# philipturner/metal-flash-attention

Hardware: NVIDIA H100
Metric: giga-FMA-instr/sec forward attn N=4096 D=128 bf16 (higher is better)
Workload: dtype bf16

## Files before the change

### metal-flash-attention_b200/csrc/kernels/sm90_ptx.cuh

```cuda
#pragma once
#include <cuda_runtime.h>
#include <stdint.h>

namespace mfa {
namespace ptx {

__device__ __forceinline__ uint32_t smem_u32(const void *p) { return static_cast<uint32_t>(__cvta_generic_to_shared(p)); }

__device__ __forceinline__ void mbar_init(uint64_t *bar, uint32_t count) {
  asm volatile("mbarrier.init.shared::cta.b64 [%0], %1;" ::"r"(smem_u32(bar)), "r"(count) : "memory");
}
__device__ __forceinline__ void fence_barrier_init() { asm volatile("fence.mbarrier_init.release.cluster;" ::: "memory"); }
__device__ __forceinline__ void fence_proxy_async_smem() { asm volatile("fence.proxy.async.shared::cta;" ::: "memory"); }

__device__ __forceinline__ void mbar_arrive(uint64_t *bar) {
  asm volatile("mbarrier.arrive.shared::cta.b64 _, [%0];" ::"r"(smem_u32(bar)) : "memory");
}
__device__ __forceinline__ void mbar_arrive_expect_tx(uint64_t *bar, uint32_t bytes) {
  asm volatile("mbarrier.arrive.expect_tx.shared::cta.b64 _, [%0], %1;" ::"r"(smem_u32(bar)), "r"(bytes) : "memory");
}
__device__ __forceinline__ void mbar_complete_tx(uint64_t *bar, uint32_t bytes) {
  asm volatile("mbarrier.complete_tx.relaxed.cta.shared::cta.b64 [%0], %1;" ::"r"(smem_u32(bar)), "r"(bytes) : "memory");
}
__device__ __forceinline__ bool mbar_try_wait(uint64_t *bar, uint32_t parity) {
  uint32_t ok;
  asm volatile(
      "{\n"
      ".reg .pred P;\n"
      "mbarrier.try_wait.parity.shared::cta.b64 P, [%1], %2;\n"
      "selp.u32 %0, 1, 0, P;\n"
      "}\n"
      : "=r"(ok)
      : "r"(smem_u32(bar)), "r"(parity)
      : "memory");
  return ok != 0;
}

#ifndef MFA_MBAR_TIMEOUT_CYCLES
#define MFA_MBAR_TIMEOUT_CYCLES (8000000000ll)
#endif
__device__ __forceinline__ void mbar_wait(uint64_t *bar, uint32_t parity) {
  if (mbar_try_wait(bar, parity)) return;
  const long long start = clock64();
  uint32_t spins = 0;
  while (!mbar_try_wait(bar, parity))
    if ((++spins & 0x3ffu) == 0 && clock64() - start > MFA_MBAR_TIMEOUT_CYCLES) __trap();
}

__device__ __forceinline__ void prefetch_tensormap(const void *map) {
  asm volatile("prefetch.tensormap [%0];" ::"l"(reinterpret_cast<uint64_t>(map)) : "memory");
}
__device__ __forceinline__ void tma_load_3d(void *smem_dst, const void *map, uint64_t *bar, int32_t c0, int32_t c1,
                                            int32_t c2) {
  asm volatile(
      "cp.async.bulk.tensor.3d.shared::cluster.global.mbarrier::complete_tx::bytes [%0], [%1, {%3, %4, %5}], [%2];"
      ::"r"(smem_u32(smem_dst)), "l"(reinterpret_cast<uint64_t>(map)), "r"(smem_u32(bar)), "r"(c0), "r"(c1), "r"(c2)
      : "memory");
}

__device__ __forceinline__ uint64_t make_smem_desc_sw128(uint32_t smem_addr, uint32_t lbo_bytes, uint32_t sbo_bytes) {
  uint64_t desc = 0;
  desc |= static_cast<uint64_t>((smem_addr & 0x3FFFFu) >> 4);
  desc |= static_cast<uint64_t>((lbo_bytes >> 4) & 0x3FFFu) << 16;
  desc |= static_cast<uint64_t>((sbo_bytes >> 4) & 0x3FFFu) << 32;
  desc |= static_cast<uint64_t>(1) << 62;
  return desc;
}

__device__ __forceinline__ float ex2_approx(float x) {
  float y;
  asm("ex2.approx.ftz.f32 %0, %1;" : "=f"(y) : "f"(x));
  return y;
}
__device__ __forceinline__ uint32_t pack_bf16x2(float lo, float hi) {
  uint32_t r;
  asm("cvt.rn.bf16x2.f32 %0, %1, %2;" : "=r"(r) : "f"(hi), "f"(lo));
  return r;
}
__device__ __forceinline__ uint32_t pack_f16x2(float lo, float hi) {
  uint32_t r;
  asm("cvt.rn.f16x2.f32 %0, %1, %2;" : "=r"(r) : "f"(hi), "f"(lo));
  return r;
}
__device__ __forceinline__ uint2 e4m3x4_to_f16x4(uint32_t bytes) {
  uint2 r;
  asm("{\n"
      ".reg .b16 lo, hi;\n"
      "mov.b32 {lo, hi}, %2;\n"
      "cvt.rn.f16x2.e4m3x2 %0, lo;\n"
      "cvt.rn.f16x2.e4m3x2 %1, hi;\n"
      "}\n"
      : "=r"(r.x), "=r"(r.y)
      : "r"(bytes));
  return r;
}
__device__ __forceinline__ uint32_t f16x2_to_bf16x2(uint32_t h) {
  float lo, hi;
  asm("{\n"
      ".reg .b16 a, b;\n"
      "mov.b32 {a, b}, %2;\n"
      "cvt.f32.f16 %0, a;\n"
      "cvt.f32.f16 %1, b;\n"
      "}\n"
      : "=f"(lo), "=f"(hi)
      : "r"(h));
  return pack_bf16x2(lo, hi);
}

}
}
```

### metal-flash-attention_b200/csrc/kernels/wgmma_attention.cu

```cuda
#include <cuda_fp16.h>
#include <cuda_runtime.h>
#include <math.h>
#include <stdint.h>

#include <type_traits>

#include "attention_params.h"
#include "backward_common.cuh"
#include "device_state.h"
#include "mfa_b200.h"
#include "sm90_ptx.cuh"
#include "tma_host.h"
#include "wgmma.cuh"

namespace mfa {
namespace hop {

using namespace ptx;
using bwd::load_16bit;
using bwd::load_stat;
using bwd::store_stat;

constexpr uint32_t kWG = 128;
constexpr uint32_t kRows = 64;
constexpr uint32_t kBarBytes = 64;

__device__ __forceinline__ uint32_t frag_row(uint32_t t) { return (t / 32) * 16 + (t % 32) / 4; }

template <uint32_t ROWS>
__device__ __forceinline__ uint64_t desc_kmajor(uint32_t tile, uint32_t row0, uint32_t kk) {
  return make_smem_desc_sw128(tile + (kk >> 2) * ROWS * 128 + row0 * 128 + (kk & 3) * 32, 16, 1024);
}
template <uint32_t ROWS>
__device__ __forceinline__ uint64_t desc_mnmajor(uint32_t tile, uint32_t kk, uint32_t c0) {
  return make_smem_desc_sw128(tile + c0 * ROWS * 128 + kk * 16 * 128, ROWS * 128, 1024);
}

template <uint32_t DCH, uint32_t N, bool kBF16, uint32_t ROWS_A>
__device__ __forceinline__ void mma_ss(float (&acc)[N / 2], uint32_t sA, uint32_t a0, uint32_t sB) {
#pragma unroll
  for (uint32_t kk = 0; kk < DCH * 4; ++kk)
    Wgmma<N, kBF16>::ss(acc, desc_kmajor<ROWS_A>(sA, a0, kk), desc_kmajor<N>(sB, 0, kk), kk > 0);
}

template <bool kBF16>
__device__ __forceinline__ uint32_t pack2(float lo, float hi) {
  return kBF16 ? pack_bf16x2(lo, hi) : pack_f16x2(lo, hi);
}
template <bool kBF16, int NR>
__device__ __forceinline__ void a_frag(const float (&s)[NR], uint32_t kk, uint32_t (&a)[4]) {
  a[0] = pack2<kBF16>(s[8 * kk + 0], s[8 * kk + 1]);
  a[1] = pack2<kBF16>(s[8 * kk + 2], s[8 * kk + 3]);
  a[2] = pack2<kBF16>(s[8 * kk + 4], s[8 * kk + 5]);
  a[3] = pack2<kBF16>(s[8 * kk + 6], s[8 * kk + 7]);
}

__device__ __forceinline__ uint8_t *align1024(uint8_t *p) {
  return reinterpret_cast<uint8_t *>((reinterpret_cast<uintptr_t>(p) + 1023) & ~uintptr_t(1023));
}

template <uint32_t RESIDENT, uint32_t TILE>
struct SmemLayout {
  static constexpr uint32_t kResidentBytes = RESIDENT, kStageBytes = 2 * TILE;
  static constexpr uint32_t kBarOffset = RESIDENT + 2 * kStageBytes;
  static constexpr uint32_t kSmemBytes = 1024 + kBarOffset + kBarBytes;
};

template <class Smem, bool kRelease = false>
struct Ring {
  uint8_t *base;
  uint64_t *bar;

  __device__ __forceinline__ explicit Ring(uint8_t *smem)
      : base(align1024(smem)), bar(reinterpret_cast<uint64_t *>(base + Smem::kBarOffset)) {}
  __device__ __forceinline__ uint8_t *stage(uint32_t n) const {
    return base + Smem::kResidentBytes + (n & 1) * Smem::kStageBytes;
  }

  __device__ __forceinline__ void init() const {
    if (threadIdx.x == 0) {
      for (int i = 0; i < 3; ++i) mbar_init(&bar[i], 1);
      if constexpr (kRelease)
        for (int i = 3; i < 5; ++i) mbar_init(&bar[i], 2);
      fence_barrier_init();
    }
    __syncthreads();
  }
  template <class Load>
  __device__ __forceinline__ void load(uint32_t n, uint32_t s, const Load &issue) const {
    mbar_arrive_expect_tx(&bar[1 + s], Smem::kStageBytes);
    issue(n, stage(s), &bar[1 + s]);
  }
  template <class Resident, class Load>
  __device__ __forceinline__ void start(const Resident &load_resident, uint32_t total, const Load &load) const {
    if (threadIdx.x != 0) return;
    mbar_arrive_expect_tx(&bar[0], Smem::kResidentBytes);
    load_resident(base, &bar[0]);
    for (uint32_t n = 0; n < 2 && n < total; ++n) this->load(n, n, load);
  }
  __device__ __forceinline__ void wait_resident() const { mbar_wait(&bar[0], 0); }
  __device__ __forceinline__ void wait(uint32_t n) const { mbar_wait(&bar[1 + (n & 1)], (n >> 1) & 1); }
  template <class Load>
  __device__ __forceinline__ void release_and_refill(uint32_t n, uint32_t total, const Load &load) const {
    __syncthreads();
    if (threadIdx.x == 0 && n + 2 < total) this->load(n + 2, n & 1, load);
  }
  __device__ __forceinline__ void release(uint32_t n) const {
    if (threadIdx.x % kWG == 0) mbar_arrive(&bar[3 + (n & 1)]);
  }
  template <class Load>
  __device__ __forceinline__ void refill(uint32_t n, uint32_t total, const Load &load) const {
    if (threadIdx.x == 0 && n + 2 < total) {
      mbar_wait(&bar[3 + (n & 1)], (n >> 1) & 1);
      this->load(n + 2, n & 1, load);
    }
  }
};

template <uint32_t DCH, uint32_t ROWS>
__device__ __forceinline__ void load_tile(uint8_t *dst, const CUtensorMap *map, uint64_t *bar, uint32_t row0,
                                          uint32_t head) {
#pragma unroll
  for (uint32_t c = 0; c < DCH; ++c) tma_load_3d(dst + c * ROWS * 128, map, bar, c * 64, row0, head);
}

template <int N>
__device__ __forceinline__ void zero(float (&d)[N]) {
#pragma unroll
  for (int i = 0; i < N; ++i) d[i] = 0.f;
}

template <uint32_t DCH, uint32_t ROWS, uint32_t kThreads>
__device__ __forceinline__ void zero_rows(uint8_t *tile, uint32_t first) {
  const uint32_t units = (ROWS - first) * 8;
  for (uint32_t i = threadIdx.x; i < DCH * units; i += kThreads) {
    const uint32_t c = i / units;
    reinterpret_cast<uint4 *>(tile + c * ROWS * 128 + first * 128)[i - c * units] = make_uint4(0u, 0u, 0u, 0u);
  }
}
template <uint32_t DCH, uint32_t ROWS, uint32_t kThreads>
__device__ __forceinline__ void zero_row_range(uint8_t *tile, uint32_t first, uint32_t end) {
  const uint32_t units = (end - first) * 8;
  for (uint32_t i = threadIdx.x; i < DCH * units; i += kThreads) {
    const uint32_t c = i / units;
    reinterpret_cast<uint4 *>(tile + c * ROWS * 128 + first * 128)[i - c * units] = make_uint4(0u, 0u, 0u, 0u);
  }
}

template <int NR>
__device__ __forceinline__ void store_acc(const float (&acc)[NR], float *out, uint32_t row0, uint32_t limit, uint32_t col0,
                                          uint32_t D, float inv0, float inv1) {
  const uint32_t t = threadIdx.x % kWG;
  const uint32_t r = row0 + frag_row(t);
#pragma unroll
  for (int i = 0; i < NR / 4; ++i) {
    const uint32_t col = col0 + 8 * i + 2 * (t % 4);
    if (col >= D) continue;
    if (r < limit)
      *reinterpret_cast<float2 *>(out + static_cast<size_t>(r) * D + col) = make_float2(acc[4 * i] * inv0, acc[4 * i + 1] * inv0);
    if (r + 8 < limit)
      *reinterpret_cast<float2 *>(out + static_cast<size_t>(r + 8) * D + col) =
          make_float2(acc[4 * i + 2] * inv1, acc[4 * i + 3] * inv1);
  }
}

template <uint32_t BN, bool kCausal>
__device__ __forceinline__ uint32_t key_blocks(uint32_t row_base, uint32_t rows, uint32_t R, uint32_t C, int delta,
                                               uint32_t kb0, uint32_t per_split) {
  if constexpr (!kCausal) {
    return min((C + BN - 1) / BN - kb0, per_split);
  } else {
    const int last_key = static_cast<int>(min(row_base + rows, R)) - 1 + delta;
    const int end = last_key < 0 ? 0 : min(static_cast<int>((C + BN - 1) / BN), last_key / static_cast<int>(BN) + 1);
    return static_cast<uint32_t>(max(0, min(end, static_cast<int>(kb0 + per_split)) - static_cast<int>(kb0)));
  }
}

template <uint32_t BM>
// ... 378 lines not shown
        first = kept.x * box;
        end = min(kept.y * box, end);
      }
      convert_fp8_kv<DCH, BN, Cfg::kThreads, kBF16>(ring.stage(j), ring.base + Cfg::Fp8Smem::kConvertedOffset, first, end);
      fence_proxy_async_smem();
      __syncthreads();
      if (tid == 0 && j + 2 < blocks) ring.load(j + 2, j & 1, load_kv);
    } else if constexpr (kLayout == KVLayout::kPaged && kBand) {
      const uint2 kept = band_boxes(kb0 + j, BN, box, band_lo, min(band_hi, static_cast<int>(span.C) - 1));
      const uint32_t first = kept.x * box, end = min(kept.y * box, span.C - (kb0 + j) * BN);
      if (first > 0 || end < BN) {
        zero_row_range<DCH, BN, Cfg::kThreads>(ring.stage(j), 0, first);
        zero_row_range<DCH, BN, Cfg::kThreads>(ring.stage(j), end, BN);
        zero_row_range<DCH, BN, Cfg::kThreads>(ring.stage(j) + Cfg::kKVBytes, 0, first);
        zero_row_range<DCH, BN, Cfg::kThreads>(ring.stage(j) + Cfg::kKVBytes, end, BN);
        fence_proxy_async_smem();
        __syncthreads();
      }
    } else if (kVarlen && ((kBand || kSplit ? kb0 : 0) + j + 1) * BN > span.C) {
      const uint32_t kb = (kBand || kSplit ? kb0 : 0) + j;
      zero_rows<DCH, BN, Cfg::kThreads>(ring.stage(j), span.C - kb * BN);
      zero_rows<DCH, BN, Cfg::kThreads>(ring.stage(j) + Cfg::kKVBytes, span.C - kb * BN);
      fence_proxy_async_smem();
      __syncthreads();
    }
    const uint32_t sK = smem_u32(kFp8 ? ring.base + Cfg::Fp8Smem::kConvertedOffset : ring.stage(j)), sV = sK + Cfg::kKVBytes;
    float sc[BN / 2];
    zero(sc);
    wgmma_fence();
    mma_ss<DCH, BN, kBF16, Cfg::kTileM>(sc, sQ, wg * kRows, sK);
    wgmma_commit();
    if constexpr (kRelease)
      if (j > 0) ring.refill(j - 1, blocks, load_kv);
    wgmma_wait<0>();
    fence_regs(sc);

    if ((kb0 + j + 1) * BN > span.C) mask_past_edge(sc, (kb0 + j) * BN, span.C);
    if constexpr (kSplit) {
      const int key0 = static_cast<int>((kb0 + j) * BN);
      const int64_t lower = kBand ? static_cast<int64_t>(delta) - band.left : -(int64_t(1) << 40);
      const int64_t upper = static_cast<int64_t>(delta) + (kBand ? band.right : 0);
      if ((kBand || kCausal) && crosses_band(key0, key0 + static_cast<int>(BN) - 1, static_cast<int>(row_base),
                                             static_cast<int>(row_base + tile_rows) - 1, lower, upper))
        mask_rows_outside_band(sc, qrow0, qrow1, key0, lower, upper);
    } else if constexpr (kBand) {
      const int key0 = static_cast<int>((kb0 + j) * BN), row = static_cast<int>(row_base + wg * kRows + frag_row(t));
      const int64_t lower = static_cast<int64_t>(delta) - band.left, upper = static_cast<int64_t>(delta) + band.right;
      if (crosses_band(key0, key0 + static_cast<int>(BN) - 1, static_cast<int>(row_base),
                       static_cast<int>(row_base + Cfg::kTileM) - 1, lower, upper))
        mask_outside_band<false>(sc, row, key0, lower, upper);
    } else if constexpr (kCausal) {
      const int key0 = static_cast<int>((kb0 + j) * BN);
      if (crosses_diagonal(key0 + static_cast<int>(BN) - 1, static_cast<int>(row_base), delta))
        mask_past_diagonal<false>(sc, static_cast<int>(row_base + wg * kRows + frag_row(t)), key0, delta);
    }
    float r0 = -INFINITY, r1 = -INFINITY;
#pragma unroll
    for (uint32_t i = 0; i < BN / 8; ++i) {
      r0 = fmaxf(r0, fmaxf(sc[4 * i], sc[4 * i + 1]));
      r1 = fmaxf(r1, fmaxf(sc[4 * i + 2], sc[4 * i + 3]));
    }
    r0 = fmaxf(r0, __shfl_xor_sync(0xffffffffu, r0, 1));
    r0 = fmaxf(r0, __shfl_xor_sync(0xffffffffu, r0, 2));
    r1 = fmaxf(r1, __shfl_xor_sync(0xffffffffu, r1, 1));
    r1 = fmaxf(r1, __shfl_xor_sync(0xffffffffu, r1, 2));
    const float mn0 = fmaxf(m0, r0 * scale_log2), mn1 = fmaxf(m1, r1 * scale_log2);
    const float ref0 = kCausal && mn0 == -INFINITY ? 0.f : mn0, ref1 = kCausal && mn1 == -INFINITY ? 0.f : mn1;
    const float a0 = ex2_approx(m0 - ref0), a1 = ex2_approx(m1 - ref1);
    m0 = mn0;
    m1 = mn1;
    l0 *= a0;
    l1 *= a1;
#pragma unroll
    for (uint32_t i = 0; i < NO / 8; ++i) {
      o[4 * i] *= a0;
      o[4 * i + 1] *= a0;
      o[4 * i + 2] *= a1;
      o[4 * i + 3] *= a1;
    }
#pragma unroll
    for (uint32_t i = 0; i < BN / 8; ++i) {
      sc[4 * i] = ex2_approx(fmaf(sc[4 * i], scale_log2, -ref0));
      sc[4 * i + 1] = ex2_approx(fmaf(sc[4 * i + 1], scale_log2, -ref0));
      sc[4 * i + 2] = ex2_approx(fmaf(sc[4 * i + 2], scale_log2, -ref1));
      sc[4 * i + 3] = ex2_approx(fmaf(sc[4 * i + 3], scale_log2, -ref1));
      l0 += sc[4 * i] + sc[4 * i + 1];
      l1 += sc[4 * i + 2] + sc[4 * i + 3];
    }
    wgmma_fence();
#pragma unroll
    for (uint32_t kk = 0; kk < BN / 16; ++kk) {
      uint32_t a[4];
      a_frag<kBF16>(sc, kk, a);
      Wgmma<NO, kBF16>::rs(o, a, desc_mnmajor<BN>(sV, kk, 0), 1);
      if constexpr (DCH == 1) {
        wgmma_commit();
        wgmma_wait<0>();
      }
    }
    wgmma_commit();
    wgmma_wait<0>();
    fence_regs(o);
    if constexpr (kFp8)
      __syncthreads();
    else if constexpr (kRelease)
      ring.release(j);
    else
      ring.release_and_refill(j, blocks, load_kv);
  }

  l0 += __shfl_xor_sync(0xffffffffu, l0, 1);
  l0 += __shfl_xor_sync(0xffffffffu, l0, 2);
  l1 += __shfl_xor_sync(0xffffffffu, l1, 1);
  l1 += __shfl_xor_sync(0xffffffffu, l1, 2);
  if constexpr (kSplit) {
    const uint32_t split = blockIdx.x % sp.splits;
#pragma unroll
    for (uint32_t h = 0; h < 2; ++h) {
      const uint32_t trow = trow0 + 8 * h, r = row_base + trow % tile_rows, qh = head * hpt + trow / tile_rows;
      if (trow >= hpt * tile_rows || r >= span.R) continue;
      const float l = h ? l1 : l0, mrow = h ? m1 : m0;
      const float inv = l == 0.f ? 0.f : (kFp8 ? (1.0f / l) * v_scale : 1.0f / l);
      const size_t row = (sp.splits == 1 ? static_cast<size_t>(qh) : static_cast<size_t>(split) * sp.batch + qh) * R +
                         span.q0 + r;
      float *out = (sp.splits == 1 ? O : sp.O_part) + row * D;
#pragma unroll
      for (int i = 0; i < NO / 8; ++i) {
        const uint32_t col = 8 * i + 2 * (t % 4);
        if (col < D)
          *reinterpret_cast<float2 *>(out + col) = make_float2(o[4 * i + 2 * h] * inv, o[4 * i + 2 * h + 1] * inv);
      }
      if (t % 4 == 0)
        store_stat(sp.splits == 1 ? L : sp.L_part, row, sp.splits == 1 ? l_prec : FP32,
                   l == 0.f ? (sp.splits == 1 ? INFINITY : -INFINITY) : mrow + log2f(l));
    }
    return;
  }
  const uint32_t row0 = row_base + wg * kRows;
  const size_t slice = static_cast<size_t>(blockIdx.z) * sp.batch + head;
  float *Oout = sp.splits == 1 ? O + (static_cast<size_t>(head) * R + span.q0) * D : sp.O_part + slice * R * D;
  const bool empty0 = (kCausal || kVarlen) && l0 == 0.f, empty1 = (kCausal || kVarlen) && l1 == 0.f;
  store_acc(o, Oout, row0, span.R, 0, D, empty0 ? 0.f : 1.0f / l0, empty1 ? 0.f : 1.0f / l1);
  if (t % 4 == 0) {
    const uint32_t r = row0 + frag_row(t);
    void *Lout = sp.splits == 1 ? L : sp.L_part;
    const int prec = sp.splits == 1 ? l_prec : FP32;
    const size_t hb = (sp.splits == 1 ? static_cast<size_t>(head) : slice) * R + span.q0;
    const float none = sp.splits == 1 ? INFINITY : -INFINITY;
    if (r < span.R) store_stat(Lout, hb + r, prec, empty0 ? none : m0 + log2f(l0));
    if (r + 8 < span.R) store_stat(Lout, hb + r + 8, prec, empty1 ? none : m1 + log2f(l1));
  }
}

template <uint32_t DCH, bool kBF16, bool kCausal>
__global__ void __launch_bounds__(2 * kWG, 1)
    attention_forward_wgmma(const __grid_constant__ CUtensorMap mapQ, const __grid_constant__ CUtensorMap mapK,
                            const __grid_constant__ CUtensorMap mapV, const __grid_constant__ FwdArgs a) {
  forward_body<DCH, kBF16, kCausal, KVLayout::kFixed>(mapQ, mapK, mapV, a);
}

template <uint32_t DCH, bool kBF16, bool kCausal>
__global__ void __launch_bounds__(2 * kWG, 1)
    packed_forward_wgmma(const __grid_constant__ CUtensorMap mapQ, const __grid_constant__ CUtensorMap mapK,
                         const __grid_constant__ CUtensorMap mapV, const __grid_constant__ FwdArgs a) {
  forward_body<DCH, kBF16, kCausal, KVLayout::kPacked>(mapQ, mapK, mapV, a);
}

template <uint32_t DCH, bool kBF16, bool kCausal>
__global__ void __launch_bounds__(2 * kWG, 1)
    paged_forward_wgmma(const __grid_constant__ CUtensorMap mapQ, const __grid_constant__ CUtensorMap mapK,
                        const __grid_constant__ CUtensorMap mapV, const __grid_constant__ FwdArgs a) {
  forward_body<DCH, kBF16, kCausal, KVLayout::kPaged>(mapQ, mapK, mapV, a);
}

template <uint32_t DCH, bool kBF16>
__global__ void __launch_bounds__(2 * kWG, 1)
    band_forward_wgmma(const __grid_constant__ CUtensorMap mapQ, const __grid_constant__ CUtensorMap mapK,
                       const __grid_constant__ CUtensorMap mapV, const __grid_constant__ FwdArgs a) {
  forward_body<DCH, kBF16, true, KVLayout::kFixed, true>(mapQ, mapK, mapV, a);
}
template <uint32_t DCH, bool kBF16>
__global__ void __launch_bounds__(2 * kWG, 1)
    band_forward_packed_wgmma(const __grid_constant__ CUtensorMap mapQ, const __grid_constant__ CUtensorMap mapK,
                              const __grid_constant__ CUtensorMap mapV, const __grid_constant__ FwdArgs a) {
  forward_body<DCH, kBF16, true, KVLayout::kPacked, true>(mapQ, mapK, mapV, a);
}
template <uint32_t DCH, bool kBF16>
__global__ void __launch_bounds__(2 * kWG, 1)
    band_forward_paged_wgmma(const __grid_constant__ CUtensorMap mapQ, const __grid_constant__ CUtensorMap mapK,
                             const __grid_constant__ CUtensorMap mapV, const __grid_constant__ FwdArgs a) {
  forward_body<DCH, kBF16, true, KVLayout::kPaged, true>(mapQ, mapK, mapV, a);
}

template <uint32_t DCH, bool kBF16, bool kCausal>
__global__ void __launch_bounds__(2 * kWG, 1)
    split_forward_packed_wgmma(const __grid_constant__ CUtensorMap mapQ, const __grid_constant__ CUtensorMap mapK,
                               const __grid_constant__ CUtensorMap mapV, const __grid_constant__ FwdArgs a) {
  forward_body<DCH, kBF16, kCausal, KVLayout::kPacked, false, true>(mapQ, mapK, mapV, a);
}
template <uint32_t DCH, bool kBF16, bool kCausal>
__global__ void __launch_bounds__(2 * kWG, DCH == 1 && !kCausal ? 2 : 1)
    split_forward_paged_wgmma(const __grid_constant__ CUtensorMap mapQ, const __grid_constant__ CUtensorMap mapK,
                              const __grid_constant__ CUtensorMap mapV, const __grid_constant__ FwdArgs a) {
  forward_body<DCH, kBF16, kCausal, KVLayout::kPaged, false, true>(mapQ, mapK, mapV, a);
}
template <uint32_t DCH, bool kBF16>
__global__ void __launch_bounds__(2 * kWG, 1)
    split_forward_packed_band_wgmma(const __grid_constant__ CUtensorMap mapQ, const __grid_constant__ CUtensorMap mapK,
                                    const __grid_constant__ CUtensorMap mapV, const __grid_constant__ FwdArgs a) {
  forward_body<DCH, kBF16, true, KVLayout::kPacked, true, true>(mapQ, mapK, mapV, a);
}
template <uint32_t DCH, bool kBF16>
__global__ void __launch_bounds__(2 * kWG, 1)
    split_forward_paged_band_wgmma(const __grid_constant__ CUtensorMap mapQ, const __grid_constant__ CUtensorMap mapK,
                                   const __grid_constant__ CUtensorMap mapV, const __grid_constant__ FwdArgs a) {
  forward_body<DCH, kBF16, true, KVLayout::kPaged, true, true>(mapQ, mapK, mapV, a);
}

template <uint32_t DCH, bool kBF16, bool kCausal>
__global__ void __launch_bounds__(2 * kWG, 1)
    fp8_kv_forward_wgmma(const __grid_constant__ CUtensorMap mapQ, const __grid_constant__ CUtensorMap mapK,
                         const __grid_constant__ CUtensorMap mapV, const __grid_constant__ FwdArgs a) {
  forward_body<DCH, kBF16, kCausal, KVLayout::kPaged, false, true, true>(mapQ, mapK, mapV, a);
}
template <uint32_t DCH, bool kBF16>
__global__ void __launch_bounds__(2 * kWG, 1)
    fp8_kv_window_forward_wgmma(const __grid_constant__ CUtensorMap mapQ, const __grid_constant__ CUtensorMap mapK,
                                const __grid_constant__ CUtensorMap mapV, const __grid_constant__ FwdArgs a) {
  forward_body<DCH, kBF16, true, KVLayout::kPaged, true, true, true>(mapQ, mapK, mapV, a);
}

template <uint32_t DCH>
struct QCfg {
  static constexpr uint32_t kWarpgroups = DCH == 4 ? 1 : 2;
  static constexpr uint32_t kThreads = kWarpgroups * kWG, kTileM = kWarpgroups * kRows, BN = 64;
  static constexpr uint32_t kPar = kTileM, kTrav = BN, kQueryBoxRows = kTileM, kKeyBoxRows = BN;
  static constexpr uint32_t kQBytes = DCH * kTileM * 128, kKVBytes = DCH * BN * 128;
  using Smem = SmemLayout<2 * kQBytes, kKVBytes>;
};

struct BwdArgs {
  const float *O;
  const void *dO;
  const void *L;
  void *Dterm;
  float *dQ, *dK, *dV;
  size_t split_stride;
  uint32_t blocks_per_split;
  uint32_t R, C, D;
  float scale, scale_log2;
  int l_prec, d_prec, dO_bf16;
  int delta;
  uint32_t group;
};

template <uint32_t DCH, bool kBF16, bool kConvertDO, bool kCausal, bool kVarlen, bool kBand = false>
__device__ __forceinline__ void backward_query_body(const CUtensorMap &mapQ, const CUtensorMap &mapdO,
                                                    const CUtensorMap &mapK, const CUtensorMap &mapV, const BwdArgs &a,
                                                    const Sequences &seq, const Band &band = Band{}) {
  using Cfg = QCfg<DCH>;
  constexpr uint32_t NO = DCH * 64, BN = Cfg::BN;
  extern __shared__ uint8_t smem_raw[];
  const Ring<typename Cfg::Smem> ring(smem_raw);
  const uint32_t tid = threadIdx.x, wg = tid / kWG, t = tid % kWG;
  const uint32_t tile = kCausal ? gridDim.x - 1 - blockIdx.x : blockIdx.x;
  const uint32_t head = blockIdx.y, row_base = tile * Cfg::kTileM, kv_head = head / a.group;
  SequenceSpan span{0, a.R, 0, a.C};
  int delta = a.delta;
  uint32_t kb0, per_split;
  if constexpr (kVarlen) {
    span = sequence_span(seq, blockIdx.z);
    if (row_base >= span.R) return;
    delta = static_cast<int>(span.C) - static_cast<int>(span.R);
    kb0 = 0;
    per_split = (span.C + BN - 1) / BN;
  } else {
    kb0 = blockIdx.z * a.blocks_per_split;
    per_split = a.blocks_per_split;
  }
  uint32_t blocks;
  if constexpr (kBand) {
    blocks = band_split(band_key_blocks<BN>(row_base, Cfg::kTileM, span.R, span.C, delta, band),
                        kVarlen ? 0u : blockIdx.z, per_split, &kb0);
  } else {
    blocks = key_blocks<BN, kCausal>(row_base, Cfg::kTileM, span.R, span.C, delta, kb0, per_split);
  }

  auto load_kv = [&](uint32_t j, uint8_t *dst, uint64_t *bar) {
    load_tile<DCH, BN>(dst, &mapK, bar, span.k0 + (kb0 + j) * BN, kv_head);
    load_tile<DCH, BN>(dst + Cfg::kKVBytes, &mapV, bar, span.k0 + (kb0 + j) * BN, kv_head);
  };
  ring.init();
  ring.start(
      [&](uint8_t *dst, uint64_t *bar) {
        load_tile<DCH, Cfg::kTileM>(dst, &mapQ, bar, span.q0 + row_base, head);
        load_tile<DCH, Cfg::kTileM>(dst + Cfg::kQBytes, &mapdO, bar, span.q0 + row_base, head);
      },
      blocks, load_kv);

  const uint32_t row0 = row_base + wg * kRows;
  const uint32_t r = row0 + frag_row(t);
  const size_t hb = static_cast<size_t>(head) * a.R + span.q0;
  float Dr[2], Lr[2];
#pragma unroll
  for (uint32_t h = 0; h < 2; ++h) {
    const uint32_t rc = min(r + 8 * h, span.R - 1);
    const float *Orow = a.O + (hb + rc) * a.D;
    const size_t drow = (hb + rc) * a.D;
    float part = 0.f;
    for (uint32_t d = 2 * (t % 4); d < a.D; d += 8) {
      const float2 ov = *reinterpret_cast<const float2 *>(Orow + d);
      part = fmaf(ov.x, load_16bit(a.dO, drow + d, a.dO_bf16), part);
// ... 220 lines not shown
#pragma unroll
    for (uint32_t j = 0; j < BM / 8; ++j)
#pragma unroll
      for (uint32_t e = 0; e < 4; ++e) {
        const uint32_t k = 4 * j + e, c = 2 * j + (e & 1);
        const float p = q0 + 8 * j + (e & 1) < span.R ? ex2_approx(fmaf(st[k], a.scale_log2, -Lq[c])) : 0.f;
        st[k] = p;
        dpt[k] = p * fmaf(dpt[k], a.scale, -Dq[c]);
      }
    wgmma_fence();
#pragma unroll
    for (uint32_t kk = 0; kk < BM / 16; ++kk) {
      uint32_t f[4];
      a_frag<kBF16>(st, kk, f);
      Wgmma<NA, kBF16>::rs(dv, f, desc_mnmajor<BM>(sdO, kk, nchunk), 1);
      a_frag<kBF16>(dpt, kk, f);
      Wgmma<NA, kBF16>::rs(dk, f, desc_mnmajor<BM>(sQ, kk, nchunk), 1);
    }
    wgmma_commit();
    wgmma_wait<0>();
    fence_regs(dv);
    fence_regs(dk);
    ring.release_and_refill(n, total, load_qd);
    if (++i == blocks) {
      i = 0;
      hb += a.R;
    }
  }
  const size_t kb = (static_cast<size_t>(kv_head) * a.C + span.k0) * a.D;
  const uint32_t row0 = key_base + krow, col0 = nchunk * 64;
  const size_t split = kVarlen ? 0 : blockIdx.z * a.split_stride;
  store_acc(dv, a.dV + split + kb, row0, span.C, col0, a.D, 1.f, 1.f);
  store_acc(dk, a.dK + split + kb, row0, span.C, col0, a.D, 1.f, 1.f);
}

template <uint32_t DCH, bool kBF16, bool kConvertDO, bool kCausal>
__global__ void __launch_bounds__(2 * kWG, 1)
    attention_backward_key_value_wgmma(const __grid_constant__ CUtensorMap mapQ, const __grid_constant__ CUtensorMap mapdO,
                                       const __grid_constant__ CUtensorMap mapK, const __grid_constant__ CUtensorMap mapV,
                                       const BwdArgs a) {
  backward_key_value_body<DCH, kBF16, kConvertDO, kCausal, false>(mapQ, mapdO, mapK, mapV, a, Sequences{});
}

template <uint32_t DCH, bool kBF16, bool kConvertDO, bool kCausal>
__global__ void __launch_bounds__(2 * kWG, 1)
    packed_backward_key_value_wgmma(const __grid_constant__ CUtensorMap mapQ,
                                              const __grid_constant__ CUtensorMap mapdO,
                                              const __grid_constant__ CUtensorMap mapK,
                                              const __grid_constant__ CUtensorMap mapV, const BwdArgs a,
                                              const Sequences seq) {
  backward_key_value_body<DCH, kBF16, kConvertDO, kCausal, true>(mapQ, mapdO, mapK, mapV, a, seq);
}

template <uint32_t DCH, bool kBF16, bool kConvertDO>
__global__ void __launch_bounds__(2 * kWG, 1)
    band_backward_key_value_wgmma(const __grid_constant__ CUtensorMap mapQ, const __grid_constant__ CUtensorMap mapdO,
                                  const __grid_constant__ CUtensorMap mapK, const __grid_constant__ CUtensorMap mapV,
                                  const BwdArgs a, const Band band) {
  backward_key_value_body<DCH, kBF16, kConvertDO, true, false, true>(mapQ, mapdO, mapK, mapV, a, Sequences{}, band);
}
template <uint32_t DCH, bool kBF16, bool kConvertDO>
__global__ void __launch_bounds__(2 * kWG, 1)
    band_backward_key_value_packed_wgmma(const __grid_constant__ CUtensorMap mapQ,
                                         const __grid_constant__ CUtensorMap mapdO,
                                         const __grid_constant__ CUtensorMap mapK,
                                         const __grid_constant__ CUtensorMap mapV, const BwdArgs a,
                                         const Sequences seq, const Band band) {
  backward_key_value_body<DCH, kBF16, kConvertDO, true, true, true>(mapQ, mapdO, mapK, mapV, a, seq, band);
}

static uint32_t chunks(uint32_t D) { return D <= 64 ? 1 : (D <= 128 ? 2 : 4); }

__global__ void __launch_bounds__(256) sum_splits(const float4 *__restrict__ part, float4 *__restrict__ out0,
                                                  float4 *__restrict__ out1, size_t quads, size_t split_stride_quads,
                                                  uint32_t splits) {
  const size_t i = static_cast<size_t>(blockIdx.x) * blockDim.x + threadIdx.x;
  if (i >= quads) return;
  const float4 *src = part + blockIdx.y * quads + i;
  float4 acc = __ldcg(src);
  for (uint32_t s = 1; s < splits; ++s) {
    const float4 v = __ldcg(src + s * split_stride_quads);
    acc.x += v.x;
    acc.y += v.y;
    acc.z += v.z;
    acc.w += v.w;
  }
  (blockIdx.y == 0 ? out0 : out1)[i] = acc;
}

static uint32_t choose_splits(uint32_t items, uint32_t total_blocks, uint32_t sm_count, uint32_t min_blocks,
                              uint32_t max_splits) {
  if (items * 2 > sm_count || min_blocks == 0) return 1;
  if (max_splits > 16) max_splits = 16;
  const uint32_t target = sm_count / items;
  uint32_t best = 1;
  for (uint32_t s = 2; s <= target && s <= max_splits; ++s)
    if (total_blocks % s == 0 && total_blocks / s >= min_blocks) best = s;
  return best;
}

static uint32_t choose_key_splits(uint64_t items, uint32_t total_blocks, uint32_t sm_count, uint32_t min_blocks,
                                  uint32_t max_splits) {
  if (items * 2 > sm_count || min_blocks == 0) return 1;
  if (max_splits > 16) max_splits = 16;
  const uint32_t target = sm_count / static_cast<uint32_t>(items);
  uint32_t best = 1;
  for (uint32_t s = 2; s <= target && s <= max_splits; ++s)
    if (total_blocks / s >= min_blocks) best = s;
  return best;
}

static uint32_t choose_blocks_per_split(uint32_t ctas, uint32_t total_blocks, uint32_t sm_count, uint32_t min_blocks,
                                        uint32_t max_splits) {
  if (ctas * 2 > sm_count || min_blocks == 0 || total_blocks < 2 * min_blocks) return total_blocks;
  if (max_splits > 8) max_splits = 8;
  uint32_t splits = sm_count / ctas;
  if (splits > max_splits) splits = max_splits;
  if (splits < 2) return total_blocks;
  uint32_t per = (total_blocks + splits - 1) / splits;
  if (per < min_blocks) per = min_blocks;
  return per;
}

template <class F>
static auto with_chunks(uint32_t D, F f) {
  switch (chunks(D)) {
    case 1: return f(std::integral_constant<uint32_t, 1>());
    case 2: return f(std::integral_constant<uint32_t, 2>());
    default: return f(std::integral_constant<uint32_t, 4>());
  }
}

template <typename Kernel>
static cudaError_t prepare(Kernel kernel, uint32_t smem) {
  return ensure_max_dynamic_smem(reinterpret_cast<const void *>(kernel), smem, current_device());
}

struct TensorMaps {
  CUtensorMap Q, dO, K, V;
};
template <class Cfg>
static cudaError_t make_maps(const AttentionParams &p, bool with_dO, TensorMaps *m) {
  cudaError_t e;
  if ((e = make_tensor_map_16bit(&m->Q, p.buf[sQ], p.R, p.D, p.batch, Cfg::kQueryBoxRows)) != cudaSuccess) return e;
  if (with_dO &&
      (e = make_tensor_map_16bit(&m->dO, p.buf[sdO], p.R, p.D, p.batch, Cfg::kQueryBoxRows)) != cudaSuccess)
    return e;
  const uint32_t kv_heads = p.batch / p.group;
  if ((e = make_tensor_map_16bit(&m->K, p.buf[sK], p.C, p.D, kv_heads, Cfg::kKeyBoxRows)) != cudaSuccess) return e;
  return make_tensor_map_16bit(&m->V, p.buf[sV], p.C, p.D, kv_heads, Cfg::kKeyBoxRows);
}

using ForwardKernel = void (*)(const CUtensorMap, const CUtensorMap, const CUtensorMap, const FwdArgs);
template <uint32_t DCH, bool kBF16, bool kCausal>
static ForwardKernel forward_kernel(KVLayout layout, bool band, bool split, bool fp8) {
  if (fp8) return band ? fp8_kv_window_forward_wgmma<DCH, kBF16> : fp8_kv_forward_wgmma<DCH, kBF16, kCausal>;
  if (split && layout == KVLayout::kPaged)
    return band ? split_forward_paged_band_wgmma<DCH, kBF16> : split_forward_paged_wgmma<DCH, kBF16, kCausal>;
  if (split) return band ? split_forward_packed_band_wgmma<DCH, kBF16> : split_forward_packed_wgmma<DCH, kBF16, kCausal>;
  if (layout == KVLayout::kPaged) return band ? band_forward_paged_wgmma<DCH, kBF16> : paged_forward_wgmma<DCH, kBF16, kCausal>;
  if (layout == KVLayout::kPacked)
    return band ? band_forward_packed_wgmma<DCH, kBF16> : packed_forward_wgmma<DCH, kBF16, kCausal>;
  return band ? band_forward_wgmma<DCH, kBF16> : attention_forward_wgmma<DCH, kBF16, kCausal>;
}

template <uint32_t DCH, bool kBF16, bool kCausal>
static cudaError_t launch_forward(const AttentionParams &p, const ForwardCall &call, const WgmmaPlan &plan,
                                  cudaStream_t stream) {
  using Cfg = FwdCfg<DCH>;
  constexpr uint32_t kSmemBytes = Cfg::Smem::kSmemBytes;
  const KVLayout layout = call.pk ? KVLayout::kPaged : (call.seq ? KVLayout::kPacked : KVLayout::kFixed);
  const bool split = layout != KVLayout::kFixed && (call.fp8 || plan.splits > 1 || plan.heads_per_tile > 1);
  const ForwardKernel kernel = forward_kernel<DCH, kBF16, kCausal>(layout, call.band, split, call.fp8);
  const uint32_t hpt = plan.heads_per_tile;
  FwdArgs a{static_cast<float *>(p.buf[sO]), p.buf[sL], p.R, p.C, p.D, p.scale_log2, p.prec[sL], p.causal_offset,
            p.group, SplitArgs{plan.blocks_per_split, plan.splits, p.batch, nullptr, nullptr}, hpt,
            call.seq ? *call.seq : Sequences{}, call.pk ? *call.pk : PagedKV{}, call.band ? *call.band : Band{},
            call.fp8 ? *call.fp8 : Fp8KV{}};
  CUtensorMap mapQ, mapK, mapV;
  cudaError_t e;
  if ((e = prepare(kernel, kSmemBytes)) != cudaSuccess ||
      (e = make_tensor_map_16bit(&mapQ, p.buf[sQ], p.R, p.D, p.batch, Cfg::kTileM / hpt, hpt)) != cudaSuccess)
    return e;
  if (call.pk) {
    const uint32_t box = min(1u << call.pk->page_shift, Cfg::BN);
    auto pool = call.fp8 ? make_tensor_map_page_pool_8bit : make_tensor_map_page_pool;
    if ((e = pool(&mapK, p.buf[sK], p.C, call.pk->kv_heads, p.D, box)) != cudaSuccess ||
        (e = pool(&mapV, p.buf[sV], p.C, call.pk->kv_heads, p.D, box)) != cudaSuccess)
      return e;
  } else if ((e = make_tensor_map_16bit(&mapK, p.buf[sK], p.C, p.D, p.batch / p.group, Cfg::BN)) != cudaSuccess ||
             (e = make_tensor_map_16bit(&mapV, p.buf[sV], p.C, p.D, p.batch / p.group, Cfg::BN)) != cudaSuccess) {
    return e;
  }
  const uint64_t rows_total = static_cast<uint64_t>(p.batch) * p.R;
  if (plan.splits > 1) {
    void *ws = nullptr;
    const size_t o_elems = plan.splits * rows_total * p.D;
    if ((e = workspace_for(current_device(), stream, (o_elems + plan.splits * rows_total) * sizeof(float), &ws)) !=
        cudaSuccess)
      return e;
    a.sp.O_part = static_cast<float *>(ws);
    a.sp.L_part = a.sp.O_part + o_elems;
  }
  kernel<<<plan.grid, Cfg::kThreads, kSmemBytes, stream>>>(mapQ, mapK, mapV, a);
  if ((e = cudaGetLastError()) != cudaSuccess || plan.splits == 1) return e;
  if (layout == KVLayout::kFixed) {
    const uint64_t threads = rows_total * (p.D / 4);
    auto merge = call.band ? merge_splits<true> : merge_splits<kCausal>;
    merge<<<static_cast<uint32_t>((threads + 127) / 128), 128, 0, stream>>>(a.sp, a.O, a.L, a.l_prec, rows_total, p.D);
  } else {
    const uint64_t threads = static_cast<uint64_t>(call.pk ? call.pk->max_row : call.seq->max_row) * (p.D / 4);
    merge_sequence_splits<<<dim3(static_cast<uint32_t>((threads + 127) / 128), p.batch, plan.grid.z), 128, 0, stream>>>(
        a.sp, a.O, a.L, a.l_prec, p.R, p.D, call.pk ? call.pk->row_offsets : call.seq->row_offsets);
  }
  return cudaGetLastError();
}

static BwdArgs backward_args(const AttentionParams &p, const WgmmaPlan &plan) {
  BwdArgs a;
  a.O = static_cast<const float *>(p.buf[sO]);
  a.dO = p.buf[sdO];
  a.L = p.buf[sL];
  a.Dterm = p.buf[sD];
  a.dQ = static_cast<float *>(p.buf[sdQ]);
  a.dK = static_cast<float *>(p.buf[sdK]);
  a.dV = static_cast<float *>(p.buf[sdV]);
  a.blocks_per_split = plan.blocks_per_split;
  a.R = p.R;
  a.C = p.C;
  a.D = p.D;
  a.scale = p.scale;
  a.scale_log2 = p.scale_log2;
  a.l_prec = p.prec[sL];
  a.d_prec = p.prec[sD];
  a.dO_bf16 = p.prec[sdO] == BF16;
  a.delta = p.causal_offset;
  a.group = p.group;
  return a;
}

using OutputSlot = float *BwdArgs::*;
template <class Cfg, class Kernel, class PackedKernel, class... Extra>
static cudaError_t launch_backward(Kernel kernel, PackedKernel packed, const AttentionParams &p, const WgmmaPlan &plan,
                                   const Sequences *seq, OutputSlot out0, OutputSlot out1, size_t elems,
                                   cudaStream_t stream, const Extra &...extra) {
  constexpr uint32_t kSmemBytes = Cfg::Smem::kSmemBytes;
  const uint32_t outputs = out1 ? 2 : 1;
  TensorMaps m;
  cudaError_t e;
  if (seq) {
    if ((e = prepare(packed, kSmemBytes)) != cudaSuccess || (e = make_maps<Cfg>(p, true, &m)) != cudaSuccess) return e;
    packed<<<plan.grid, Cfg::kThreads, kSmemBytes, stream>>>(m.Q, m.dO, m.K, m.V, backward_args(p, plan), *seq,
                                                             extra...);
    return cudaGetLastError();
  }
  if ((e = prepare(kernel, kSmemBytes)) != cudaSuccess || (e = make_maps<Cfg>(p, true, &m)) != cudaSuccess) return e;
  BwdArgs a = backward_args(p, plan);
  float *const dst0 = a.*out0, *const dst1 = out1 ? a.*out1 : nullptr;
  float *scratch = nullptr;
  if (plan.splits > 1) {
    void *ws = nullptr;
    if ((e = workspace_for(current_device(), stream, plan.splits * outputs * elems * sizeof(float), &ws)) != cudaSuccess)
      return e;
    scratch = static_cast<float *>(ws);
    a.split_stride = outputs * elems;
    a.*out0 = scratch;
    if (out1) a.*out1 = scratch + elems;
  }
  kernel<<<plan.grid, Cfg::kThreads, kSmemBytes, stream>>>(m.Q, m.dO, m.K, m.V, a, extra...);
  if ((e = cudaGetLastError()) != cudaSuccess || plan.splits == 1) return e;
  const size_t quads = elems / 4;
  sum_splits<<<dim3(static_cast<uint32_t>((quads + 255) / 256), outputs), 256, 0, stream>>>(
      reinterpret_cast<const float4 *>(scratch), reinterpret_cast<float4 *>(dst0), reinterpret_cast<float4 *>(dst1), quads,
      a.split_stride / 4, plan.splits);
  return cudaGetLastError();
}

template <class F>
static cudaError_t dispatch(const AttentionParams &p, bool convert_dO, F f) {
  return with_chunks(p.D, [&](auto dch) {
    auto types = [&](auto causal) {
      if (convert_dO) return f(dch, std::false_type(), std::true_type(), causal);
      if (p.prec[sQ] == BF16) return f(dch, std::true_type(), std::false_type(), causal);
      return f(dch, std::false_type(), std::false_type(), causal);
    };
    return p.causal ? types(std::true_type()) : types(std::false_type());
  });
}

}

WgmmaPlan wgmma_plan(int type, uint32_t D, uint32_t R, uint32_t C, uint32_t batch, uint32_t group, uint32_t min_blocks,
                     uint32_t max_splits, bool convert_dO, uint32_t sm_count, const Band *band) {
  WgmmaPlan p{};
  p.heads_per_tile = 1;
  auto geometry = [&](auto cfg) {
    using Cfg = decltype(cfg);
    p.threads = Cfg::kThreads;
    p.smem_bytes = Cfg::Smem::kSmemBytes;
    p.par = Cfg::kPar;
    p.trav = Cfg::kTrav;
  };
  hop::with_chunks(D, [&](auto dch) {
    constexpr uint32_t DCH = decltype(dch)::value;
    if (type == MFA_FORWARD)
      geometry(hop::FwdCfg<DCH>());
    else if (type == MFA_BACKWARD_QUERY)
      geometry(hop::QCfg<DCH>());
    else
      geometry(hop::KVCfg<DCH>());
  });
  const uint32_t padded = (D + 7) / 8 * 8, columns = hop::chunks(D) * 64;
  p.head = columns < padded ? columns : padded;

  const bool key_value = type == MFA_BACKWARD_KEY_VALUE;
  const uint32_t tiles = ((key_value ? C : R) + p.par - 1) / p.par;
  uint32_t total = ((key_value ? R : C) + p.trav - 1) / p.trav;
  if (band) {
    const uint64_t width = (static_cast<uint64_t>(p.par) + band->left + band->right + p.trav - 1) / p.trav + 1;
    if (width < total) total = static_cast<uint32_t>(width);
  }
  const uint32_t heads = key_value ? batch / group : batch;
  if (type == MFA_FORWARD) {
    p.splits = hop::choose_splits(tiles * heads, total, sm_count, min_blocks, max_splits);
    p.blocks_per_split = total / p.splits;
  } else {
    p.blocks_per_split = hop::choose_blocks_per_split(tiles * heads, total, sm_count, min_blocks, max_splits);
    p.splits = (total + p.blocks_per_split - 1) / p.blocks_per_split;
  }
  p.grid = dim3(tiles, heads, p.splits);
  p.convert_dO_first = key_value && convert_dO && static_cast<uint64_t>(tiles) * heads > sm_count;
  p.launches = 1 + (p.splits > 1 ? 1 : 0) + (p.convert_dO_first ? 1 : 0);
  return p;
}

WgmmaPlan wgmma_plan_sequences(int type, uint32_t D, uint32_t max_row, uint32_t max_column, uint32_t count,
                               uint32_t batch, uint32_t group, bool convert_dO, uint32_t sm_count) {
  WgmmaPlan p = wgmma_plan(type, D, max_row, max_column, batch, group, 0, 1, convert_dO, sm_count);
  p.grid.z = count;
  p.convert_dO_first = type == MFA_BACKWARD_KEY_VALUE && convert_dO &&
                       static_cast<uint64_t>(p.grid.x) * p.grid.y * count > sm_count;
  p.launches = 1 + (p.convert_dO_first ? 1 : 0);
  return p;
}

WgmmaPlan wgmma_plan_split(uint32_t D, uint32_t max_row, uint32_t key_bound, uint32_t count, uint32_t batch,
                           uint32_t group, uint32_t min_blocks, uint32_t max_splits, uint32_t num_splits,
                           uint32_t sm_count, const Band *band) {
  WgmmaPlan p = wgmma_plan(MFA_FORWARD, D, max_row, key_bound, batch, 1, 0, 1, false, sm_count, band);
  p.heads_per_tile = group >= 2 && group <= p.par && max_row < p.par ? group : 1;
  const uint32_t rows = p.par / p.heads_per_tile, tiles = (max_row + rows - 1) / rows;
  const uint64_t items = static_cast<uint64_t>(tiles) * (batch / p.heads_per_tile) * count;
  p.splits = num_splits ? num_splits : hop::choose_key_splits(items, p.blocks_per_split, sm_count, min_blocks, max_splits);
  p.grid = dim3(tiles * p.splits, batch / p.heads_per_tile, count);
  p.launches = 1 + (p.splits > 1 ? 1 : 0);
  return p;
}
// ... 108 lines not shown
```

Before: 314,900.

## Add warp-specialized producer/consumer forward kernel for non-causal D=128

For the fixed-layout non-causal D=128 forward path, adds a third warpgroup that acts as a dedicated TMA producer with reduced registers, feeding K and V through separate double-buffered rings with full/empty mbarriers. The two consumer warpgroups raise their register limits and overlap the next S=QK^T wgmma with the previous PV wgmma, using a ping-pong turn barrier so their tensor-core issue alternates. The aim is to hide load latency and overlap softmax with MMA, as FA3-style kernels do. It costs more barrier bookkeeping and a larger barrier region, and it relies on register reallocation being correct.

```diff
diff --git a/metal-flash-attention_b200/csrc/kernels/sm90_ptx.cuh b/metal-flash-attention_b200/csrc/kernels/sm90_ptx.cuh
--- a/metal-flash-attention_b200/csrc/kernels/sm90_ptx.cuh
+++ b/metal-flash-attention_b200/csrc/kernels/sm90_ptx.cuh
@@ -45,6 +45,27 @@
   uint32_t spins = 0;
   while (!mbar_try_wait(bar, parity))
     if ((++spins & 0x3ffu) == 0 && clock64() - start > MFA_MBAR_TIMEOUT_CYCLES) __trap();
+}
+
+template <uint32_t kRegs>
+__device__ __forceinline__ void setmaxnreg_dec() {
+  asm volatile("setmaxnreg.dec.sync.aligned.u32 %0;" ::"n"(kRegs));
+}
+template <uint32_t kRegs>
+__device__ __forceinline__ void setmaxnreg_inc() {
+  asm volatile("setmaxnreg.inc.sync.aligned.u32 %0;" ::"n"(kRegs));
+}
+
+template <uint32_t kEntryRegs>
+__device__ __forceinline__ void mbar_wait_raised(uint64_t *bar, uint32_t parity) {
+  if (__all_sync(0xffffffffu, mbar_try_wait(bar, parity))) return;
+  const long long start = clock64();
+  uint32_t spins = 0;
+  while (!__all_sync(0xffffffffu, mbar_try_wait(bar, parity)))
+    if ((++spins & 0x3ffu) == 0 && __any_sync(0xffffffffu, clock64() - start > MFA_MBAR_TIMEOUT_CYCLES)) {
+      setmaxnreg_dec<kEntryRegs>();
+      __trap();
+    }
 }
 
 __device__ __forceinline__ void prefetch_tensormap(const void *map) {
diff --git a/metal-flash-attention_b200/csrc/kernels/wgmma_attention.cu b/metal-flash-attention_b200/csrc/kernels/wgmma_attention.cu
--- a/metal-flash-attention_b200/csrc/kernels/wgmma_attention.cu
+++ b/metal-flash-attention_b200/csrc/kernels/wgmma_attention.cu
@@ -23,7 +23,7 @@
 
 constexpr uint32_t kWG = 128;
 constexpr uint32_t kRows = 64;
-constexpr uint32_t kBarBytes = 64;
+constexpr uint32_t kBarBytes = 128;
 
 __device__ __forceinline__ uint32_t frag_row(uint32_t t) { return (t / 32) * 16 + (t % 32) / 4; }
 
@@ -708,12 +708,195 @@
   }
 }
 
+template <uint32_t DCH, bool kCausal>
+constexpr bool kWarpSpecialized = DCH == 2 && !kCausal;
+template <uint32_t DCH, bool kCausal>
+constexpr uint32_t kFixedForwardThreads = kWarpSpecialized<DCH, kCausal> ? 3 * kWG : 2 * kWG;
+
+template <uint32_t DCH, bool kBF16>
+__device__ __forceinline__ void forward_ws_body(const CUtensorMap &mapQ, const CUtensorMap &mapK, const CUtensorMap &mapV,
+                                                const FwdArgs &a) {
+  using Cfg = FwdCfg<DCH>;
+  using Smem = typename Cfg::Smem;
+  constexpr uint32_t NO = DCH * 64, BN = Cfg::BN, kStages = 2;
+  static_assert(Smem::kBarOffset == Cfg::kQBytes + 2 * kStages * Cfg::kKVBytes, "Q, then the K ring, then the V ring");
+  static_assert((1 + 4 * kStages + 2) * sizeof(uint64_t) <= kBarBytes, "the barriers fit");
+  extern __shared__ uint8_t smem_raw[];
+  uint8_t *const base = align1024(smem_raw);
+  uint8_t *const sK0 = base + Cfg::kQBytes, *const sV0 = sK0 + kStages * Cfg::kKVBytes;
+  uint64_t *const q_full = reinterpret_cast<uint64_t *>(base + Smem::kBarOffset);
+  uint64_t *const k_full = q_full + 1, *const k_empty = k_full + kStages, *const v_full = k_empty + kStages,
+                  *const v_empty = v_full + kStages, *const turn = v_empty + kStages;
+  const uint32_t tid = threadIdx.x, wg = __shfl_sync(0xffffffffu, tid / kWG, 0), t = tid % kWG;
+  const uint32_t head = blockIdx.y, row_base = blockIdx.x * Cfg::kTileM, kv_head = head / a.group;
+  const uint32_t kb0 = blockIdx.z * a.sp.blocks_per_split;
+  const uint32_t blocks = key_blocks<BN, false>(row_base, Cfg::kTileM, a.R, a.C, a.delta, kb0, a.sp.blocks_per_split);
+  if (tid == 0) {
+    prefetch_tensormap(&mapQ);
+    prefetch_tensormap(&mapK);
+    prefetch_tensormap(&mapV);
+    mbar_init(q_full, 1);
+    for (uint32_t s = 0; s < kStages; ++s) {
+      mbar_init(&k_full[s], 1);
+      mbar_init(&v_full[s], 1);
+      mbar_init(&k_empty[s], 8);
+      mbar_init(&v_empty[s], 8);
+    }
+    mbar_init(&turn[0], 4);
+    mbar_init(&turn[1], 4);
+    fence_barrier_init();
+  }
+  __syncthreads();
+
+  if (wg == 0) {
+    setmaxnreg_dec<24>();
+    if (tid != 0 || blocks == 0) return;
+    mbar_arrive_expect_tx(q_full, Cfg::kQBytes);
+    load_tile<DCH, Cfg::kTileM>(base, &mapQ, q_full, row_base, head);
+    auto load = [&](uint32_t j, uint8_t *ring, uint64_t *full, uint64_t *empty, const CUtensorMap *map) {
+      const uint32_t s = j % kStages;
+      if (j >= kStages) mbar_wait(&empty[s], (j / kStages - 1) & 1);
+      mbar_arrive_expect_tx(&full[s], Cfg::kKVBytes);
+      load_tile<DCH, BN>(ring + s * Cfg::kKVBytes, map, &full[s], (kb0 + j) * BN, kv_head);
+    };
+    load(0, sK0, k_full, k_empty, &mapK);
+    for (uint32_t j = 1; j < blocks; ++j) {
+      load(j, sK0, k_full, k_empty, &mapK);
+      load(j - 1, sV0, v_full, v_empty, &mapV);
+    }
+    load(blocks - 1, sV0, v_full, v_empty, &mapV);
+    return;
+  }
+
+  setmaxnreg_inc<240>();
+  constexpr uint32_t kEntryRegs = 65536 / (3 * kWG) / 8 * 8;
+  const uint32_t cw = wg - 1;
+  const uint32_t sQ = smem_u32(base);
+  const float scale_log2 = a.scale_log2;
+  float o[NO / 2];
+  zero(o);
+  float sc[BN / 2];
+  float m0 = -INFINITY, m1 = -INFINITY, l0 = 0.f, l1 = 0.f;
+  auto release = [&](uint64_t *empty) {
+    if (t % 32 == 0) mbar_arrive(empty);
+  };
+  auto issue_s = [&](uint32_t j) {
+    mma_ss<DCH, BN, kBF16, Cfg::kTileM>(sc, sQ, cw * kRows, smem_u32(sK0 + (j % kStages) * Cfg::kKVBytes));
+    wgmma_commit();
+  };
+  auto issue_pv = [&](uint32_t j, const uint32_t (&p)[BN / 16][4]) {
+    const uint32_t sV = smem_u32(sV0 + (j % kStages) * Cfg::kKVBytes);
+#pragma unroll
+    for (uint32_t kk = 0; kk < BN / 16; ++kk) Wgmma<NO, kBF16>::rs(o, p[kk], desc_mnmajor<BN>(sV, kk, 0), 1);
+    wgmma_commit();
+  };
+  auto pack = [&](uint32_t (&p)[BN / 16][4]) {
+#pragma unroll
+    for (uint32_t kk = 0; kk < BN / 16; ++kk) a_frag<kBF16>(sc, kk, p[kk]);
+  };
+  auto softmax = [&](uint32_t j, float &a0, float &a1) {
+    if ((kb0 + j + 1) * BN > a.C) mask_past_edge(sc, (kb0 + j) * BN, a.C);
+    float r0 = -INFINITY, r1 = -INFINITY;
+#pragma unroll
+    for (uint32_t i = 0; i < BN / 8; ++i) {
+      r0 = fmaxf(r0, fmaxf(sc[4 * i], sc[4 * i + 1]));
+      r1 = fmaxf(r1, fmaxf(sc[4 * i + 2], sc[4 * i + 3]));
+    }
+    r0 = fmaxf(r0, __shfl_xor_sync(0xffffffffu, r0, 1));
+    r0 = fmaxf(r0, __shfl_xor_sync(0xffffffffu, r0, 2));
+    r1 = fmaxf(r1, __shfl_xor_sync(0xffffffffu, r1, 1));
+    r1 = fmaxf(r1, __shfl_xor_sync(0xffffffffu, r1, 2));
+    const float mn0 = fmaxf(m0, r0 * scale_log2), mn1 = fmaxf(m1, r1 * scale_log2);
+    a0 = ex2_approx(m0 - mn0);
+    a1 = ex2_approx(m1 - mn1);
+    m0 = mn0;
+    m1 = mn1;
+    l0 *= a0;
+    l1 *= a1;
+#pragma unroll
+    for (uint32_t i = 0; i < BN / 8; ++i) {
+      sc[4 * i] = ex2_approx(fmaf(sc[4 * i], scale_log2, -mn0));
+      sc[4 * i + 1] = ex2_approx(fmaf(sc[4 * i + 1], scale_log2, -mn0));
+      sc[4 * i + 2] = ex2_approx(fmaf(sc[4 * i + 2], scale_log2, -mn1));
+      sc[4 * i + 3] = ex2_approx(fmaf(sc[4 * i + 3], scale_log2, -mn1));
+      l0 += sc[4 * i] + sc[4 * i + 1];
+      l1 += sc[4 * i + 2] + sc[4 * i + 3];
+    }
+  };
+
+  auto wait_v = [&](uint32_t j) { mbar_wait_raised<kEntryRegs>(&v_full[j % kStages], (j / kStages) & 1); };
+  if (blocks > 0) {
+    float a0, a1;
+    uint32_t p[BN / 16][4];
+    mbar_wait_raised<kEntryRegs>(q_full, 0);
+    mbar_wait_raised<kEntryRegs>(&k_full[0], 0);
+    wgmma_fence();
+    issue_s(0);
+    wgmma_wait<0>();
+    fence_regs(sc);
+    release(&k_empty[0]);
+    softmax(0, a0, a1);
+    wait_v(0);
+    for (uint32_t j = 1; j < blocks; ++j) {
+      mbar_wait_raised<kEntryRegs>(&k_full[j % kStages], (j / kStages) & 1);
+      pack(p);
+      if (cw == 1 || j > 1) mbar_wait_raised<kEntryRegs>(&turn[cw], (cw == 1 ? j - 1 : j - 2) & 1);
+      wgmma_fence();
+      issue_s(j);
+      issue_pv(j - 1, p);
+      if (t % 32 == 0) mbar_arrive(&turn[1 - cw]);
+      wgmma_wait<1>();
+      fence_regs(sc);
+      release(&k_empty[j % kStages]);
+      softmax(j, a0, a1);
+      wait_v(j);
+      wgmma_wait<0>();
+      fence_regs(o);
+      release(&v_empty[(j - 1) % kStages]);
+#pragma unroll
+      for (uint32_t i = 0; i < NO / 8; ++i) {
+        o[4 * i] *= a0;
+        o[4 * i + 1] *= a0;
+        o[4 * i + 2] *= a1;
+        o[4 * i + 3] *= a1;
+      }
+    }
+    pack(p);
+    wgmma_fence();
+    issue_pv(blocks - 1, p);
+    wgmma_wait<0>();
+    fence_regs(o);
+  }
+
+  l0 += __shfl_xor_sync(0xffffffffu, l0, 1);
+  l0 += __shfl_xor_sync(0xffffffffu, l0, 2);
+  l1 += __shfl_xor_sync(0xffffffffu, l1, 1);
+  l1 += __shfl_xor_sync(0xffffffffu, l1, 2);
+  const uint32_t row0 = row_base + cw * kRows;
+  const SplitArgs &sp = a.sp;
+  const size_t slice = static_cast<size_t>(blockIdx.z) * sp.batch + head;
+  float *Oout = sp.splits == 1 ? a.O + static_cast<size_t>(head) * a.R * a.D : sp.O_part + slice * a.R * a.D;
+  store_acc(o, Oout, row0, a.R, 0, a.D, 1.0f / l0, 1.0f / l1);
+  if (t % 4 == 0) {
+    const uint32_t r = row0 + frag_row(t);
+    void *Lout = sp.splits == 1 ? a.L : sp.L_part;
+    const int prec = sp.splits == 1 ? a.l_prec : FP32;
+    const size_t hb = (sp.splits == 1 ? static_cast<size_t>(head) : slice) * a.R;
+    if (r < a.R) store_stat(Lout, hb + r, prec, m0 + log2f(l0));
+    if (r + 8 < a.R) store_stat(Lout, hb + r + 8, prec, m1 + log2f(l1));
+  }
+}
+
 template <uint32_t DCH, bool kBF16, bool kCausal>
-__global__ void __launch_bounds__(2 * kWG, 1)
+__global__ void __launch_bounds__(kFixedForwardThreads<DCH, kCausal>, 1)
     attention_forward_wgmma(const __grid_constant__ CUtensorMap mapQ, const __grid_constant__ CUtensorMap mapK,
                             const __grid_constant__ CUtensorMap mapV, const __grid_constant__ FwdArgs a) {
-  forward_body<DCH, kBF16, kCausal, KVLayout::kFixed>(mapQ, mapK, mapV, a);
-}
+  if constexpr (kWarpSpecialized<DCH, kCausal>)
+    forward_ws_body<DCH, kBF16>(mapQ, mapK, mapV, a);
+  else
+    forward_body<DCH, kBF16, kCausal, KVLayout::kFixed>(mapQ, mapK, mapV, a);
+}
+
 
 template <uint32_t DCH, bool kBF16, bool kCausal>
 __global__ void __launch_bounds__(2 * kWG, 1)
@@ -1240,16 +1423,26 @@
 }
 
 using ForwardKernel = void (*)(const CUtensorMap, const CUtensorMap, const CUtensorMap, const FwdArgs);
+struct ForwardLaunch {
+  ForwardKernel kernel;
+  uint32_t threads;
+};
 template <uint32_t DCH, bool kBF16, bool kCausal>
-static ForwardKernel forward_kernel(KVLayout layout, bool band, bool split, bool fp8) {
-  if (fp8) return band ? fp8_kv_window_forward_wgmma<DCH, kBF16> : fp8_kv_forward_wgmma<DCH, kBF16, kCausal>;
+static ForwardLaunch forward_kernel(KVLayout layout, bool band, bool split, bool fp8) {
+  constexpr uint32_t kThreads = FwdCfg<DCH>::kThreads;
+  if (fp8) return {band ? fp8_kv_window_forward_wgmma<DCH, kBF16> : fp8_kv_forward_wgmma<DCH, kBF16, kCausal>, kThreads};
   if (split && layout == KVLayout::kPaged)
-    return band ? split_forward_paged_band_wgmma<DCH, kBF16> : split_forward_paged_wgmma<DCH, kBF16, kCausal>;
-  if (split) return band ? split_forward_packed_band_wgmma<DCH, kBF16> : split_forward_packed_wgmma<DCH, kBF16, kCausal>;
-  if (layout == KVLayout::kPaged) return band ? band_forward_paged_wgmma<DCH, kBF16> : paged_forward_wgmma<DCH, kBF16, kCausal>;
+    return {band ? split_forward_paged_band_wgmma<DCH, kBF16> : split_forward_paged_wgmma<DCH, kBF16, kCausal>,
+            kThreads};
+  if (split)
+    return {band ? split_forward_packed_band_wgmma<DCH, kBF16> : split_forward_packed_wgmma<DCH, kBF16, kCausal>,
+            kThreads};
+  if (layout == KVLayout::kPaged)
+    return {band ? band_forward_paged_wgmma<DCH, kBF16> : paged_forward_wgmma<DCH, kBF16, kCausal>, kThreads};
   if (layout == KVLayout::kPacked)
-    return band ? band_forward_packed_wgmma<DCH, kBF16> : packed_forward_wgmma<DCH, kBF16, kCausal>;
-  return band ? band_forward_wgmma<DCH, kBF16> : attention_forward_wgmma<DCH, kBF16, kCausal>;
+    return {band ? band_forward_packed_wgmma<DCH, kBF16> : packed_forward_wgmma<DCH, kBF16, kCausal>, kThreads};
+  if (band) return {band_forward_wgmma<DCH, kBF16>, kThreads};
+  return {attention_forward_wgmma<DCH, kBF16, kCausal>, kFixedForwardThreads<DCH, kCausal>};
 }
 
 template <uint32_t DCH, bool kBF16, bool kCausal>
@@ -1259,7 +1452,8 @@
   constexpr uint32_t kSmemBytes = Cfg::Smem::kSmemBytes;
   const KVLayout layout = call.pk ? KVLayout::kPaged : (call.seq ? KVLayout::kPacked : KVLayout::kFixed);
   const bool split = layout != KVLayout::kFixed && (call.fp8 || plan.splits > 1 || plan.heads_per_tile > 1);
-  const ForwardKernel kernel = forward_kernel<DCH, kBF16, kCausal>(layout, call.band, split, call.fp8);
+  const ForwardLaunch launch = forward_kernel<DCH, kBF16, kCausal>(layout, call.band, split, call.fp8);
+  const ForwardKernel kernel = launch.kernel;
   const uint32_t hpt = plan.heads_per_tile;
   FwdArgs a{static_cast<float *>(p.buf[sO]), p.buf[sL], p.R, p.C, p.D, p.scale_log2, p.prec[sL], p.causal_offset,
             p.group, SplitArgs{plan.blocks_per_split, plan.splits, p.batch, nullptr, nullptr}, hpt,
@@ -1290,7 +1484,7 @@
     a.sp.O_part = static_cast<float *>(ws);
     a.sp.L_part = a.sp.O_part + o_elems;
   }
-  kernel<<<plan.grid, Cfg::kThreads, kSmemBytes, stream>>>(mapQ, mapK, mapV, a);
+  kernel<<<plan.grid, launch.threads, kSmemBytes, stream>>>(mapQ, mapK, mapV, a);
   if ((e = cudaGetLastError()) != cudaSuccess || plan.splits == 1) return e;
   if (layout == KVLayout::kFixed) {
     const uint64_t threads = rows_total * (p.D / 4);
```

New measurement: 324,600, median of 6. 1.03x the previous value.
